# Jeremy-Cleland/hmer-img2latex

Measured on AMD Instinct MI355X. Metric: decoded LaTeX tokens/sec at batch 256, 320x64 imgs, seq 150, higher is better.
Workload: dtype f32

## Files before the change

### hmer-img2latex_amd/csrc/conv_bf16x3.hip

```cpp
#include <stdlib.h>

#include "common.h"

namespace {

#include "bf16_split.inc.h"

typedef float f32x16 __attribute__((ext_vector_type(16)));

constexpr int CH = 16;
constexpr int CO_BLK = 64;
constexpr int W_SLAB_U4 = 9 * 3 * 2 * CO_BLK;
constexpr int W_PHASE_U4 = W_SLAB_U4 / 3;

template <int WX> struct Tile3 {
    static constexpr int TR = (4 / WX) * 4, TC = WX * 16;
    static constexpr int IR = TR + 2, IC = TC + 2;
    static constexpr int ICP = WX == 2 ? 36 : (WX == 1 ? 20 : 68);
    static constexpr int ROW16 = 2 * ICP;
    static constexpr int IN_U4 = 3 * IR * ROW16;
};

constexpr unsigned FIX_HDR = 64;
constexpr unsigned FIX_CAP = 1u << 20;
constexpr float FIX_TOL = 0x1p-13f;

__device__ __forceinline__ void pool_window(float a0, float a1, float a2, float a3, float bv, float& outv, int& bi, bool& near) {
    float best = a0;
    bi = 0;
    if (a1 > best) { best = a1; bi = 1; }
    if (a2 > best) { best = a2; bi = 2; }
    if (a3 > best) { best = a3; bi = 3; }
    const float pre = best + bv;
    outv = fmaxf(pre, 0.f);
    const float scale = fmaxf(fmaxf(fabsf(best), fabsf(bv)), 1e-30f);
    const float thr = FIX_TOL * scale;
    const float d0 = best - a0, d1 = best - a1, d2 = best - a2, d3 = best - a3;
    const bool tie = (d0 > 0.f && d0 <= thr) || (d1 > 0.f && d1 <= thr) || (d2 > 0.f && d2 <= thr) || (d3 > 0.f && d3 <= thr);
    near = fabsf(pre) <= thr || (tie && pre > 0.f);
}
__device__ __forceinline__ void fix_append(unsigned* fix, size_t o) {
    const unsigned at = atomicAdd(fix, 1u);
    if (at < FIX_CAP) fix[FIX_HDR + at] = (unsigned)o;
}

__global__ void conv_pack3_kernel(const float* __restrict__ w, bf16_t* __restrict__ wp, int Cin, int Cout, int n_chunks,
                                  size_t total, int flip, unsigned* __restrict__ fix) {
    const size_t idx = (size_t)blockIdx.x * blockDim.x + threadIdx.x;
    if (idx == 0 && fix) fix[0] = 0;
    if (idx >= total) return;
    size_t r = idx;
    const int j = (int)(r % 8); r /= 8;
    const int co_l = (int)(r % CO_BLK); r /= CO_BLK;
    const int lh = (int)(r % 2); r /= 2;
    const int tap = (int)(r % 9); r /= 9;
    const int chunk = (int)(r % n_chunks);
    const int cb = (int)(r / n_chunks);
    const int co = cb * CO_BLK + co_l, ci = chunk * CH + 8 * lh + j;
    const float v = (co < Cout && ci < Cin) ? (flip ? w[((size_t)ci * Cout + co) * 9 + (8 - tap)] : w[((size_t)co * Cin + ci) * 9 + tap]) : 0.f;
    bf16_t s[3];
    split3(v, s[0], s[1], s[2]);
    const size_t slab = ((size_t)cb * n_chunks + chunk) * (size_t)W_SLAB_U4 * 8;
#pragma unroll
    for (int sp = 0; sp < 3; ++sp)
        wp[slab + ((((size_t)tap * 3 + sp) * 2 + lh) * CO_BLK + co_l) * 8 + j] = s[sp];
}

template <int WX, bool FULL = false, bool AM = false, int NT = 2>
__global__ __launch_bounds__(256, 2) void conv3x3_bf16x3_kernel(
    const float* __restrict__ x, const bf16_t* __restrict__ wpack, const float* __restrict__ bias,
    float* __restrict__ y, unsigned char* __restrict__ amax, int Cin, int H, int W, int Cout, int Hp, int Wp,
    int tiles_x, int n_chunks, int tiles_per_img, int n_items, int items_per_wg, unsigned* __restrict__ fix) {
    typedef Tile3<WX> TL;
    constexpr int PR = TL::TR / 2, PC = TL::TC / 2;
    constexpr bool LO = FULL && NT == 1;
    __shared__ __attribute__((aligned(16))) uint4 in_s[TL::IN_U4];
    __shared__ __attribute__((aligned(16))) uint4 w_s[W_PHASE_U4];
    __shared__ float out_s[CO_BLK * 65];
    __shared__ unsigned char am_s[AM ? CO_BLK * 68 : 4];

    const int tid = threadIdx.x, lane = tid & 63, wave = tid >> 6;
    const int wy = wave / WX, wx = wave % WX;
    constexpr int CO_W = 32 * NT;
    const int co_blocks_g = (Cout + CO_W - 1) / CO_W;
    const int lin = blockIdx.x, within = lin % (8 * co_blocks_g);
    const int cb = within >> 3;
    const int walk = (lin / (8 * co_blocks_g)) * 8 + (within & 7);
    const int i = lane & 31, h = lane >> 5;
    const int dx = i & 1, dy = (i >> 1) & 1, pp = i >> 2;
    const int a_base = ((wy * 4 + dy) * 2 + h) * TL::ICP + wx * 16 + 2 * pp + dx;
    const int b_base = h * CO_BLK + i + (NT == 1 ? (cb & 1) * 32 : 0);
    const uint4* wp_cb = reinterpret_cast<const uint4*>(wpack) + (size_t)(NT == 1 ? cb >> 1 : cb) * n_chunks * W_SLAB_U4;
    const int HW = H * W;

    constexpr int NP = TL::IR * 2 * TL::IC;
    constexpr int NE = (NP + 255) / 256;
    constexpr int NWV = (W_PHASE_U4 + 255) / 256;
    constexpr int SPLIT_U4 = TL::IR * TL::ROW16;
    int loff[NE], p_r[NE], p_col[NE], p_lh[NE];
#pragma unroll
    for (int e = 0; e < NE; ++e) {
        const int idx = tid + e * 256;
        p_col[e] = idx % TL::IC;
        p_lh[e] = (idx / TL::IC) & 1;
        p_r[e] = idx / (2 * TL::IC);
        loff[e] = idx < NP ? (p_r[e] * 2 + p_lh[e]) * TL::ICP + p_col[e] : -1;
    }
    const float* f_xb = x;
    int goff[NE];
    unsigned okmask = 0;
    auto setup_fetch = [&](int item) {
        const int fb = item / tiles_per_img, ft = item - fb * tiles_per_img;
        const int fty = ft / tiles_x, ftx = ft - fty * tiles_x;
        const int fy0 = fty * TL::TR, fx0 = ftx * TL::TC;
        f_xb = x + (size_t)fb * Cin * HW;
        okmask = 0;
#pragma unroll
        for (int e = 0; e < NE; ++e) {
            const int iy = fy0 - 1 + p_r[e], ix = fx0 - 1 + p_col[e];
            goff[e] = (8 * p_lh[e] * H + iy) * W + ix;
            if (loff[e] >= 0 && iy >= 0 && iy < H && ix >= 0 && ix < W) okmask |= 1u << e;
        }
    };
    float xin[NE][8];
    uint4 win[NWV];
    auto fetch_x = [&](int chunk) {
        const float* xc = f_xb + (size_t)chunk * CH * HW;
#pragma unroll
        for (int e = 0; e < NE; ++e) {
            const bool ok = (okmask >> e) & 1u;
#pragma unroll
            for (int j = 0; j < 8; ++j) xin[e][j] = ok ? xc[goff[e] + j * HW] : 0.f;
        }
    };
    auto fetch_w = [&](int phase) {
        const uint4* wsrc = wp_cb + (size_t)phase * W_PHASE_U4;
#pragma unroll
        for (int e = 0; e < NWV; ++e) {
            const int idx = tid + e * 256;
            win[e] = idx < W_PHASE_U4 ? wsrc[idx] : make_uint4(0, 0, 0, 0);
        }
    };
    auto commit_x = [&]() {
#pragma unroll
        for (int e = 0; e < NE; ++e) {
            if (loff[e] >= 0) {
                unsigned s[3][4];
#pragma unroll
                for (int j = 0; j < 4; ++j) split3_pair(xin[e][2 * j], xin[e][2 * j + 1], s[0][j], s[1][j], s[2][j]);
#pragma unroll
                for (int sp = 0; sp < 3; ++sp)
                    in_s[loff[e] + sp * SPLIT_U4] = make_uint4(s[sp][0], s[sp][1], s[sp][2], s[sp][3]);
            }
        }
    };
    auto commit_w = [&]() {
#pragma unroll
        for (int e = 0; e < NWV; ++e) {
            const int idx = tid + e * 256;
            if (idx < W_PHASE_U4) w_s[idx] = win[e];
        }
    };

    const int n_phases = 3 * n_chunks;
    const int it0 = walk * items_per_wg, it_end = min(it0 + items_per_wg, n_items);
    if (it0 >= n_items) return;
    setup_fetch(it0);
    fetch_x(0);
    fetch_w(0);
    for (int it = it0; it < it_end; ++it) {
        const int b = it / tiles_per_img, tl = it - b * tiles_per_img;
        const int ty = tl / tiles_x, tx = tl - ty * tiles_x;
        const int y0 = ty * TL::TR, x0 = tx * TL::TC;
        f32x16 acc[2][NT];
        f32x16 acc_lo[LO ? 2 : 1];
#pragma unroll
        for (int m = 0; m < 2; ++m)
#pragma unroll
            for (int n = 0; n < NT; ++n)
#pragma unroll
                for (int r = 0; r < 16; ++r) acc[m][n][r] = 0.f;
        if constexpr (LO) {
#pragma unroll
            for (int m = 0; m < 2; ++m)
#pragma unroll
                for (int r = 0; r < 16; ++r) acc_lo[m][r] = 0.f;
        }

        for (int chunk = 0; chunk < n_chunks; ++chunk) {
#pragma unroll
            for (int ky = 0; ky < 3; ++ky) {
                __syncthreads();
                if (ky == 0) commit_x();
                commit_w();
                __syncthreads();
                if (chunk * 3 + ky + 1 < n_phases) fetch_w(chunk * 3 + ky + 1);
                else if (it + 1 < it_end) fetch_w(0);
                if (ky == 0) {
                    if (chunk + 1 < n_chunks) fetch_x(chunk + 1);
                    else if (it + 1 < it_end) { setup_fetch(it + 1); fetch_x(0); }
                }
#pragma unroll
                for (int kx = 0; kx < 3; ++kx) {
                    i16x8_t a[2][3], bw[NT][3];
#pragma unroll
                    for (int m = 0; m < 2; ++m)
#pragma unroll
                        for (int sp = 0; sp < 3; ++sp) {
                            const uint4 t = in_s[a_base + (sp * TL::IR + m * 2 + ky) * TL::ROW16 + kx];
                            a[m][sp] = *reinterpret_cast<const i16x8_t*>(&t);
                        }
#pragma unroll
                    for (int n = 0; n < NT; ++n)
#pragma unroll
                        for (int sp = 0; sp < 3; ++sp) {
                            const uint4 t = w_s[b_base + ((kx * 3 + sp) * 2) * CO_BLK + n * 32];
                            bw[n][sp] = *reinterpret_cast<const i16x8_t*>(&t);
                        }
                    constexpr int TI[6] = {0, 1, 2, 0, 1, 0}, TJ[6] = {2, 1, 0, 1, 0, 0};
#pragma unroll
                    for (int t = 0; t < 6; ++t)
#pragma unroll
                        for (int m = 0; m < 2; ++m)
#pragma unroll
                            for (int n = 0; n < NT; ++n) {
                                if constexpr (LO) {
                                    f32x16& dst = t < 5 ? acc_lo[m] : acc[m][n];
                                    dst = __builtin_amdgcn_mfma_f32_32x32x16_bf16(a[m][TI[t]], bw[n][TJ[t]], dst, 0, 0, 0);
                                } else {
                                    acc[m][n] = __builtin_amdgcn_mfma_f32_32x32x16_bf16(a[m][TI[t]], bw[n][TJ[t]], acc[m][n], 0, 0, 0);
                                }
                            }
                }
            }
        }

        const int py0 = y0 >> 1, px0 = x0 >> 1;
        if constexpr (LO) {
#pragma unroll
            for (int m = 0; m < 2; ++m) acc[m][0] += acc_lo[m];
        }
        if constexpr (FULL) {
#pragma unroll
            for (int n = 0; n < NT; ++n) {
                const int co = cb * CO_W + n * 32 + i;
                if (co >= Cout) continue;
#pragma unroll
                for (int m = 0; m < 2; ++m) {
                    const int py = py0 + wy * 2 + m;
#pragma unroll
                    for (int q = 0; q < 4; ++q) {
                        const int px = px0 + wx * 8 + 2 * q + h;
#pragma unroll
                        for (int ry = 0; ry < 2; ++ry) {
                            const int Y = 2 * py + ry, X = 2 * px;
                            if (Y < H && X + 1 < W)
                                *reinterpret_cast<float2*>(y + (((size_t)b * Cout + co) * H + Y) * W + X) =
                                    make_float2(acc[m][n][4 * q + 2 * ry], acc[m][n][4 * q + 2 * ry + 1]);
                        }
                    }
                }
            }
            continue;
        }
        if ((Wp & 3) == 0 && py0 + PR <= Hp && px0 + PC <= Wp && (cb + 1) * CO_BLK <= Cout) {
#pragma unroll
            for (int n = 0; n < NT; ++n) {
                const float bv = bias[cb * CO_BLK + n * 32 + i];
#pragma unroll
                for (int m = 0; m < 2; ++m)
#pragma unroll
                    for (int q = 0; q < 4; ++q) {
                        const int pos = (wy * 2 + m) * PC + wx * 8 + 2 * q + h;
                        if constexpr (AM) {
                            float ov;
                            int bi;
                            bool near;
                            pool_window(acc[m][n][4 * q], acc[m][n][4 * q + 1], acc[m][n][4 * q + 2], acc[m][n][4 * q + 3], bv, ov, bi, near);
                            out_s[(n * 32 + i) * 65 + pos] = ov;
                            am_s[(n * 32 + i) * 68 + pos] = (unsigned char)bi;
                            if (near && fix)
                                fix_append(fix, (((size_t)b * Cout + cb * CO_BLK + n * 32 + i) * Hp + py0 + wy * 2 + m) * Wp + px0 + wx * 8 + 2 * q + h);
                        } else {
                            const float v = fmaxf(fmaxf(acc[m][n][4 * q], acc[m][n][4 * q + 1]),
                                                  fmaxf(acc[m][n][4 * q + 2], acc[m][n][4 * q + 3])) + bv;
                            out_s[(n * 32 + i) * 65 + pos] = fmaxf(v, 0.f);
                        }
                    }
            }
            __syncthreads();
            for (int idx = tid; idx < CO_BLK * 16; idx += 256) {
                constexpr int XG = PC / 4;
                const int x4 = idx % XG, py = (idx / XG) % PR, co_l = idx >> 4;
                const float* sp = &out_s[co_l * 65 + py * PC + 4 * x4];
                const size_t o = (((size_t)b * Cout + cb * CO_BLK + co_l) * Hp + py0 + py) * Wp + px0 + 4 * x4;
                *reinterpret_cast<float4*>(y + o) = make_float4(sp[0], sp[1], sp[2], sp[3]);
                if constexpr (AM) *reinterpret_cast<uchar4*>(amax + o) = *reinterpret_cast<const uchar4*>(&am_s[co_l * 68 + py * PC + 4 * x4]);
            }
            continue;
        }
#pragma unroll
        for (int n = 0; n < NT; ++n) {
            const int co = cb * CO_BLK + n * 32 + i;
            if (co >= Cout) continue;
            const float bv = bias[co];
#pragma unroll
            for (int m = 0; m < 2; ++m) {
                const int py = py0 + wy * 2 + m;
                if (py >= Hp) continue;
                const size_t rowoff = (((size_t)b * Cout + co) * Hp + py) * Wp;
#pragma unroll
                for (int q = 0; q < 4; ++q) {
                    const int px = px0 + wx * 8 + 2 * q + h;
                    float ov;
                    int bi;
                    bool near;
                    pool_window(acc[m][n][4 * q], acc[m][n][4 * q + 1], acc[m][n][4 * q + 2], acc[m][n][4 * q + 3], bv, ov, bi, near);
                    if (px < Wp) {
                        y[rowoff + px] = ov;
                        if (amax) amax[rowoff + px] = (unsigned char)bi;
                        if (AM && near && fix) fix_append(fix, rowoff + px);
                    }
                }
            }
        }
    }
}


template <int CIN, bool AM = false>
__global__ __launch_bounds__(256, 4) void conv3x3_smallk_bf16x3_kernel(
    const float* __restrict__ x, const float* __restrict__ w, const float* __restrict__ bias, float* __restrict__ y,
    unsigned char* __restrict__ amax, int H, int W, int Cout, int Hp, int Wp, int tiles_x, int tiles_per_part,
    unsigned* __restrict__ fix) {
    constexpr int RS = 48;
    constexpr int PLANE = 10 * RS;
    __shared__ __attribute__((aligned(16))) uint2 img[3 * PLANE];
    __shared__ float out_s[32 * 65];
    __shared__ unsigned char am_s[AM ? 32 * 68 : 4];

    const int tid = threadIdx.x, lane = tid & 63, wave = tid >> 6;
    const int wy = wave >> 1, wx = wave & 1;
    const int i = lane & 31, h = lane >> 5;
    const int cbs = (Cout + 31) / 32;
    const int cb = blockIdx.x % cbs, b = blockIdx.z;
    const int tx_begin = (blockIdx.x / cbs) * tiles_per_part, tx_end = min(tiles_x, tx_begin + tiles_per_part);
    const int y0 = blockIdx.y * 8;

    i16x8_t bw[3][3];
    {
        const int co = cb * 32 + i;
#pragma unroll
        for (int s = 0; s < 3; ++s) {
            unsigned pk[3][4];
#pragma unroll
            for (int j = 0; j < 4; ++j) {
                const int tap = 4 * s + 2 * h + (j >> 1), c0 = 2 * (j & 1);
                const bool okt = tap < 9 && co < Cout;
                const float v0 = (okt && c0 < CIN) ? w[((size_t)co * CIN + c0) * 9 + tap] : 0.f;
                const float v1 = (okt && c0 + 1 < CIN) ? w[((size_t)co * CIN + c0 + 1) * 9 + tap] : 0.f;
                split3_pair(v0, v1, pk[0][j], pk[1][j], pk[2][j]);
            }
#pragma unroll
            for (int sp = 0; sp < 3; ++sp) {
                const uint4 t = make_uint4(pk[sp][0], pk[sp][1], pk[sp][2], pk[sp][3]);
                bw[s][sp] = *reinterpret_cast<const i16x8_t*>(&t);
            }
        }
    }
    const float bv = (cb * 32 + i < Cout) ? bias[cb * 32 + i] : 0.f;

    const int pbase = (wy * 4 + ((i >> 1) & 1)) * RS + wx * 16 + 2 * (i >> 2) + (i & 1);
    int aoff[3][2];
#pragma unroll
    for (int s = 0; s < 3; ++s)
#pragma unroll
        for (int e = 0; e < 2; ++e) {
            const int tap = min(4 * s + 2 * h + e, 8);
            aoff[s][e] = pbase + (tap / 3) * RS + (tap % 3);
        }

    const float* xb = x + (size_t)b * CIN * H * W;
    const size_t HW = (size_t)H * W;
    int q_lds[2], q_col[2];
    long q_goff[2];
    bool q_rowok[2];
#pragma unroll
    for (int e = 0; e < 2; ++e) {
        const int q = tid + e * 256;
        const int r = q / 34, col = q - r * 34;
        const int iy = y0 - 1 + r;
        q_lds[e] = q < 340 ? r * RS + col : -1;
        q_col[e] = col - 1;
        q_rowok[e] = q < 340 && iy >= 0 && iy < H;
        q_goff[e] = (long)iy * W + col - 1;
    }
    float pin[2][CIN];
    auto fetch = [&](int tx) {
        const int x0 = tx * 32;
#pragma unroll
        for (int e = 0; e < 2; ++e) {
            const int ix = x0 + q_col[e];
            const bool ok = q_rowok[e] && ix >= 0 && ix < W;
#pragma unroll
            for (int c = 0; c < CIN; ++c) pin[e][c] = ok ? xb[c * HW + q_goff[e] + x0] : 0.f;
        }
    };
    fetch(tx_begin);
    for (int tx = tx_begin; tx < tx_end; ++tx) {
#pragma unroll
        for (int e = 0; e < 2; ++e) {
            if (q_lds[e] >= 0) {
                unsigned p0[3], p1[3];
                split3_pair(pin[e][0], CIN > 1 ? pin[e][CIN > 1 ? 1 : 0] : 0.f, p0[0], p0[1], p0[2]);
                split3_pair(CIN > 2 ? pin[e][CIN > 2 ? 2 : 0] : 0.f, 0.f, p1[0], p1[1], p1[2]);
#pragma unroll
                for (int sp = 0; sp < 3; ++sp) img[sp * PLANE + q_lds[e]] = make_uint2(p0[sp], p1[sp]);
            }
        }
        __syncthreads();
        if (tx + 1 < tx_end) fetch(tx + 1);
#pragma unroll 1
        for (int m = 0; m < 2; ++m) {
            f32x16 acc;
#pragma unroll
            for (int r = 0; r < 16; ++r) acc[r] = 0.f;
            constexpr int TI[5] = {0, 1, 2, 0, 1}, TJ[5] = {2, 1, 0, 1, 0};
            i16x8_t a0[3];
#pragma unroll
            for (int s = 0; s < 3; ++s) {
                i16x8_t a[3];
#pragma unroll
                for (int sp = 0; sp < 3; ++sp) {
                    const uint2 t0 = img[sp * PLANE + m * 2 * RS + aoff[s][0]];
                    const uint2 t1 = img[sp * PLANE + m * 2 * RS + aoff[s][1]];
                    const uint4 t = make_uint4(t0.x, t0.y, t1.x, t1.y);
                    a[sp] = *reinterpret_cast<const i16x8_t*>(&t);
                }
                a0[s] = a[0];
#pragma unroll
                for (int t = 0; t < 5; ++t)
                    acc = __builtin_amdgcn_mfma_f32_32x32x16_bf16(a[TI[t]], bw[s][TJ[t]], acc, 0, 0, 0);
            }
#pragma unroll
            for (int s = 0; s < 3; ++s) acc = __builtin_amdgcn_mfma_f32_32x32x16_bf16(a0[s], bw[s][0], acc, 0, 0, 0);
#pragma unroll
            for (int q = 0; q < 4; ++q) {
                const int pos = (wy * 2 + m) * 16 + wx * 8 + 2 * q + h;
                if constexpr (AM) {
                    float ov;
                    int bi;
                    bool near;
                    pool_window(acc[4 * q], acc[4 * q + 1], acc[4 * q + 2], acc[4 * q + 3], bv, ov, bi, near);
                    out_s[i * 65 + pos] = ov;
                    am_s[i * 68 + pos] = (unsigned char)bi;
                    const int fpy = (y0 >> 1) + wy * 2 + m, fpx = tx * 16 + wx * 8 + 2 * q + h;
                    if (near && fix && cb * 32 + i < Cout && fpy < Hp && fpx < Wp)
                        fix_append(fix, (((size_t)b * Cout + cb * 32 + i) * Hp + fpy) * Wp + fpx);
                } else {
                    const float v = fmaxf(fmaxf(acc[4 * q], acc[4 * q + 1]), fmaxf(acc[4 * q + 2], acc[4 * q + 3])) + bv;
                    out_s[i * 65 + pos] = fmaxf(v, 0.f);
                }
            }
        }
        __syncthreads();
        const int py0 = y0 >> 1, px0 = tx * 16;
        if ((Wp & 3) == 0 && py0 + 4 <= Hp && px0 + 16 <= Wp && (cb + 1) * 32 <= Cout) {
            for (int idx = tid; idx < 32 * 16; idx += 256) {
                const int x4 = idx & 3, py = (idx >> 2) & 3, c = idx >> 4;
                const float* sp = &out_s[c * 65 + py * 16 + 4 * x4];
                const size_t o = (((size_t)b * Cout + cb * 32 + c) * Hp + py0 + py) * Wp + px0 + 4 * x4;
                *reinterpret_cast<float4*>(y + o) = make_float4(sp[0], sp[1], sp[2], sp[3]);
                if constexpr (AM) *reinterpret_cast<uchar4*>(amax + o) = *reinterpret_cast<const uchar4*>(&am_s[c * 68 + py * 16 + 4 * x4]);
            }
        } else {
            for (int idx = tid; idx < 32 * 64; idx += 256) {
                const int px = idx & 15, py = (idx >> 4) & 3, c = idx >> 6;
                if (cb * 32 + c < Cout && py0 + py < Hp && px0 + px < Wp) {
                    const size_t o = (((size_t)b * Cout + cb * 32 + c) * Hp + py0 + py) * Wp + px0 + px;
                    y[o] = out_s[c * 65 + py * 16 + px];
                    if constexpr (AM) amax[o] = am_s[c * 68 + py * 16 + px];
                }
            }
        }
    }
}

__global__ __launch_bounds__(256) void conv_pool_fixup_kernel(const float* __restrict__ x, const float* __restrict__ w,
                                                              const float* __restrict__ bias, float* __restrict__ y,
                                                              unsigned char* __restrict__ amax, const unsigned* __restrict__ fix,
                                                              int Cin, int H, int W, int Cout, int Hp, int Wp) {
    const unsigned n = min(fix[0], FIX_CAP);
    const int lane = threadIdx.x & 63;
    for (unsigned e = blockIdx.x * 4 + (threadIdx.x >> 6); e < n; e += gridDim.x * 4) {
        const unsigned o = fix[FIX_HDR + e];
        const int px = (int)(o % Wp), py = (int)((o / Wp) % Hp);
        const int co = (int)((o / ((unsigned)Wp * Hp)) % Cout), b = (int)(o / ((unsigned)Wp * Hp * Cout));
        float s[4] = {0.f, 0.f, 0.f, 0.f};
        for (int ci = lane; ci < Cin; ci += 64) {
            const float* xp = x + ((size_t)b * Cin + ci) * H * W;
            const float* wp = w + ((size_t)co * Cin + ci) * 9;
            float win[4][4];
#pragma unroll
            for (int r = 0; r < 4; ++r)
#pragma unroll
                for (int c = 0; c < 4; ++c) {
                    const int iy = 2 * py - 1 + r, ix = 2 * px - 1 + c;
                    win[r][c] = (iy >= 0 && iy < H && ix >= 0 && ix < W) ? xp[(size_t)iy * W + ix] : 0.f;
                }
#pragma unroll
            for (int ky = 0; ky < 3; ++ky)
#pragma unroll
                for (int kx = 0; kx < 3; ++kx) {
                    const float wv = wp[ky * 3 + kx];
#pragma unroll
                    for (int q = 0; q < 4; ++q) s[q] = fmaf(win[(q >> 1) + ky][(q & 1) + kx], wv, s[q]);
                }
        }
#pragma unroll
        for (int q = 0; q < 4; ++q)
#pragma unroll
            for (int off = 32; off >= 1; off >>= 1) s[q] += __shfl_xor(s[q], off);
        if (lane == 0) {
            float best = s[0];
            int bi = 0;
#pragma unroll
            for (int q = 1; q < 4; ++q)
                if (s[q] > best) { best = s[q]; bi = q; }
            y[o] = fmaxf(best + bias[co], 0.f);
            amax[o] = (unsigned char)bi;
        }
    }
}

}

bool i2l_conv_bf16x3_applicable(int Cin, int Cout) {
    return Cin % CH == 0 && Cout % CO_BLK == 0;
}
bool i2l_conv_bf16x3_full_applicable(int Cin, int Cout) {
    return Cin % CH == 0 && (Cout % CO_BLK == 0 || Cout == 32);
}

size_t i2l_conv_bf16x3_workspace_bytes(int Cin, int Cout) {
    return i2l_align((size_t)((Cout + CO_BLK - 1) / CO_BLK) * (Cin / CH) * W_SLAB_U4 * 16);
}
size_t i2l_conv_fixlist_bytes(void) { return i2l_align((size_t)(FIX_HDR + FIX_CAP) * sizeof(unsigned)); }

namespace {
int launch_fixup(const float* x, const float* w, const float* bias, float* y, unsigned char* amax, const unsigned* fix,
                 int B, int Cin, int H, int W, int Cout, hipStream_t s) {
    if ((size_t)B * Cout * (H / 2) * (W / 2) > 0xffffffffull) return I2L_ERR_UNSUPPORTED;
    hipLaunchKernelGGL(conv_pool_fixup_kernel, dim3(512), dim3(256), 0, s, x, w, bias, y, amax, fix, Cin, H, W, Cout, H / 2, W / 2);
    I2L_CHECK_LAUNCH();
    return I2L_OK;
}
}

int i2l_conv_bf16x3_run(const float* x, const float* w, const float* bias, float* y, unsigned char* amax, int B, int Cin,
                        int H, int W, int Cout, void* workspace, size_t workspace_bytes, hipStream_t s, int full,
                        int weights_packed) {
    if (full && ((H | W) & 1)) return I2L_ERR_UNSUPPORTED;
    const size_t pack_bytes = i2l_conv_bf16x3_workspace_bytes(Cin, Cout);
    if (workspace_bytes < pack_bytes + (amax ? i2l_conv_fixlist_bytes() : 0) || !workspace) return I2L_ERR_WORKSPACE;
    unsigned* fix = amax ? reinterpret_cast<unsigned*>(static_cast<char*>(workspace) + pack_bytes) : nullptr;
    if (amax && (size_t)B * Cout * (H / 2) * (W / 2) > 0xffffffffull) return I2L_ERR_UNSUPPORTED;
    const int Hp = H / 2, Wp = W / 2;
    const int n_chunks = Cin / CH, co_blocks = (Cout + CO_BLK - 1) / CO_BLK;
    if (Cout % CO_BLK != 0 && !(full && Cout == 32)) return I2L_ERR_UNSUPPORTED;
    bf16_t* wp = static_cast<bf16_t*>(workspace);
    const size_t total = (size_t)co_blocks * n_chunks * 9 * 2 * CO_BLK * 8;
    if (!(weights_packed && !amax && !full))
    hipLaunchKernelGGL(conv_pack3_kernel, dim3((unsigned)((total + 255) / 256)), dim3(256), 0, s, w, wp, Cin, Cout,
                       n_chunks, total, full ? 1 : 0, fix);
    I2L_CHECK_LAUNCH();
    const int rows = 2 * Hp, cols = 2 * Wp;
    int wx = 2;
    long bestw = -1;
    const int cand[3] = {2, 1, 4};
    for (int c = 0; c < 3; ++c) {
        const int tr = (4 / cand[c]) * 4, tc = cand[c] * 16;
        const long cover = (long)i2l_cdiv(rows, tr) * tr * i2l_cdiv(cols, tc) * tc;
        if (bestw < 0 || cover < bestw) { bestw = cover; wx = cand[c]; }
    }
    const int tr = (4 / wx) * 4, tc = wx * 16;
    const int tiles_x = i2l_cdiv(cols, tc), tiles_y = i2l_cdiv(rows, tr);
    const int tiles_per_img = tiles_x * tiles_y;
    const long long n_items_ll = (long long)tiles_per_img * B;
    if (n_items_ll > 0x7fffffffll) return I2L_ERR_UNSUPPORTED;
    const int n_items = (int)n_items_ll;
    const int wg_blocks = full ? (Cout + 31) / 32 : co_blocks;
    int items_per_wg = (int)((n_items_ll * wg_blocks + 511) / 512);
    if (n_items_ll * wg_blocks <= 768) items_per_wg = 1;
    if (items_per_wg < 1) items_per_wg = 1;
    const int walks = i2l_cdiv(n_items, items_per_wg);
    dim3 grid((unsigned)(i2l_cdiv(walks, 8) * 8 * wg_blocks));
#define I2L_LAUNCH3(WXV)                                                                                              \
    do {                                                                                                              \
        if (full)                                                                                                     \
            hipLaunchKernelGGL((conv3x3_bf16x3_kernel<WXV, true, false, 1>), grid, dim3(256), 0, s, x, (const bf16_t*)wp, bias, y, \
                               amax, Cin, H, W, Cout, Hp, Wp, tiles_x, n_chunks, tiles_per_img, n_items, items_per_wg, fix); \
        else if (amax)                                                                                                \
            hipLaunchKernelGGL((conv3x3_bf16x3_kernel<WXV, false, true>), grid, dim3(256), 0, s, x, (const bf16_t*)wp, bias, y, \
                               amax, Cin, H, W, Cout, Hp, Wp, tiles_x, n_chunks, tiles_per_img, n_items, items_per_wg, fix); \
        else                                                                                                          \
            hipLaunchKernelGGL((conv3x3_bf16x3_kernel<WXV, false>), grid, dim3(256), 0, s, x, (const bf16_t*)wp, bias, y, \
                               amax, Cin, H, W, Cout, Hp, Wp, tiles_x, n_chunks, tiles_per_img, n_items, items_per_wg, fix); \
    } while (0)
    if (wx == 2) I2L_LAUNCH3(2);
    else if (wx == 1) I2L_LAUNCH3(1);
    else I2L_LAUNCH3(4);
#undef I2L_LAUNCH3
    I2L_CHECK_LAUNCH();
    if (amax) return launch_fixup(x, w, bias, y, amax, fix, B, Cin, H, W, Cout, s);
    return I2L_OK;
}

bool i2l_conv_smallk_applicable(int Cin, int Cout) {
    return Cin >= 1 && Cin <= 3 && Cout % 32 == 0;
}

int i2l_conv_smallk_run(const float* x, const float* w, const float* bias, float* y, unsigned char* amax, int B, int Cin,
                        int H, int W, int Cout, void* workspace, size_t workspace_bytes, hipStream_t s) {
    const int Hp = H / 2, Wp = W / 2;
    unsigned* fix = nullptr;
    if (amax) {
        if (!workspace || workspace_bytes < i2l_conv_fixlist_bytes()) return I2L_ERR_WORKSPACE;
        if ((size_t)B * Cout * Hp * Wp > 0xffffffffull) return I2L_ERR_UNSUPPORTED;
        fix = static_cast<unsigned*>(workspace);
        if (hipMemsetAsync(fix, 0, sizeof(unsigned), s) != hipSuccess) return I2L_ERR_LAUNCH;
    }
    const int tiles_x = i2l_cdiv(2 * Wp, 32), bands = i2l_cdiv(2 * Hp, 8);
    if (bands > 65535 || B > 65535) return I2L_ERR_UNSUPPORTED;
    int parts = 1;
    while (parts < tiles_x && (long)(Cout / 32) * bands * B * parts < 1536) ++parts;
    const int tiles_per_part = i2l_cdiv(tiles_x, parts);
    parts = i2l_cdiv(tiles_x, tiles_per_part);
    dim3 grid((Cout / 32) * parts, bands, B);
#define I2L_LAUNCH_SK(C, A) hipLaunchKernelGGL((conv3x3_smallk_bf16x3_kernel<C, A>), grid, dim3(256), 0, s, x, w, bias, y, amax, H, W, Cout, Hp, Wp, tiles_x, tiles_per_part, fix)
    if (amax) {
        if (Cin == 1) I2L_LAUNCH_SK(1, true);
        else if (Cin == 2) I2L_LAUNCH_SK(2, true);
        else I2L_LAUNCH_SK(3, true);
    } else {
        if (Cin == 1) I2L_LAUNCH_SK(1, false);
        else if (Cin == 2) I2L_LAUNCH_SK(2, false);
        else I2L_LAUNCH_SK(3, false);
    }
#undef I2L_LAUNCH_SK
    I2L_CHECK_LAUNCH();
    if (amax) return launch_fixup(x, w, bias, y, amax, fix, B, Cin, H, W, Cout, s);
    return I2L_OK;
}
```

Before: 40.57 million.

## Double-buffer conv output tile and defer global store to overlap with MFMA

The output staging buffers (out_s, am_s) are double-buffered so each tile's global store runs during the next tile's MFMA compute rather than serially after it. The last tile is flushed after the loop, and the fast-path store loop is unrolled into two fixed iterations per thread. This adds about 8KB of LDS per block, which may lower occupancy at the requested 4 blocks per CU. Only the small-K first conv layer is affected, which is a small part of the full decode pipeline.

```diff
diff --git a/hmer-img2latex_amd/csrc/conv_bf16x3.hip b/hmer-img2latex_amd/csrc/conv_bf16x3.hip
--- a/hmer-img2latex_amd/csrc/conv_bf16x3.hip
+++ b/hmer-img2latex_amd/csrc/conv_bf16x3.hip
@@ -336,8 +336,8 @@
     constexpr int RS = 48;
     constexpr int PLANE = 10 * RS;
     __shared__ __attribute__((aligned(16))) uint2 img[3 * PLANE];
-    __shared__ float out_s[32 * 65];
-    __shared__ unsigned char am_s[AM ? 32 * 68 : 4];
+    __shared__ float out_s[2][32 * 65];
+    __shared__ unsigned char am_s[2][AM ? 32 * 68 : 4];
 
     const int tid = threadIdx.x, lane = tid & 63, wave = tid >> 6;
     const int wy = wave >> 1, wx = wave & 1;
@@ -406,8 +406,38 @@
             for (int c = 0; c < CIN; ++c) pin[e][c] = ok ? xb[c * HW + q_goff[e] + x0] : 0.f;
         }
     };
+    auto store_tile = [&](int txs, int par) {
+        const int py0 = y0 >> 1, px0 = txs * 16;
+        const float* os = out_s[par];
+        const unsigned char* as = am_s[par];
+        int ts = tid;
+        asm volatile("" : "+v"(ts));
+        if ((Wp & 3) == 0 && py0 + 4 <= Hp && px0 + 16 <= Wp && (cb + 1) * 32 <= Cout) {
+            const int x4 = ts & 3, py = (ts >> 2) & 3;
+            const size_t t = ((size_t)(ts >> 4) * Hp + py) * Wp + 4 * x4;
+#pragma unroll
+            for (int k = 0; k < 2; ++k) {
+                const int c = (ts >> 4) + 16 * k;
+                const float* sp = &os[c * 65 + py * 16 + 4 * x4];
+                const size_t o = (((size_t)b * Cout + cb * 32 + 16 * k) * Hp + py0) * Wp + px0 + t;
+                *reinterpret_cast<float4*>(y + o) = make_float4(sp[0], sp[1], sp[2], sp[3]);
+                if constexpr (AM) *reinterpret_cast<uchar4*>(amax + o) = *reinterpret_cast<const uchar4*>(&as[c * 68 + py * 16 + 4 * x4]);
+            }
+        } else {
+            for (int idx = ts; idx < 32 * 64; idx += 256) {
+                const int px = idx & 15, py = (idx >> 4) & 3, c = idx >> 6;
+                if (cb * 32 + c < Cout && py0 + py < Hp && px0 + px < Wp) {
+                    const size_t o = (((size_t)b * Cout + cb * 32 + c) * Hp + py0 + py) * Wp + px0 + px;
+                    y[o] = os[c * 65 + py * 16 + px];
+                    if constexpr (AM) amax[o] = as[c * 68 + py * 16 + px];
+                }
+            }
+        }
+    };
+    if (tx_begin >= tx_end) return;
     fetch(tx_begin);
     for (int tx = tx_begin; tx < tx_end; ++tx) {
+        const int par = (tx - tx_begin) & 1;
 #pragma unroll
         for (int e = 0; e < 2; ++e) {
             if (q_lds[e] >= 0) {
@@ -420,6 +450,7 @@
         }
         __syncthreads();
         if (tx + 1 < tx_end) fetch(tx + 1);
+        if (tx > tx_begin) store_tile(tx - 1, par ^ 1);
 #pragma unroll 1
         for (int m = 0; m < 2; ++m) {
             f32x16 acc;
@@ -452,38 +483,20 @@
                     int bi;
                     bool near;
                     pool_window(acc[4 * q], acc[4 * q + 1], acc[4 * q + 2], acc[4 * q + 3], bv, ov, bi, near);
-                    out_s[i * 65 + pos] = ov;
-                    am_s[i * 68 + pos] = (unsigned char)bi;
+                    out_s[par][i * 65 + pos] = ov;
+                    am_s[par][i * 68 + pos] = (unsigned char)bi;
                     const int fpy = (y0 >> 1) + wy * 2 + m, fpx = tx * 16 + wx * 8 + 2 * q + h;
                     if (near && fix && cb * 32 + i < Cout && fpy < Hp && fpx < Wp)
                         fix_append(fix, (((size_t)b * Cout + cb * 32 + i) * Hp + fpy) * Wp + fpx);
                 } else {
                     const float v = fmaxf(fmaxf(acc[4 * q], acc[4 * q + 1]), fmaxf(acc[4 * q + 2], acc[4 * q + 3])) + bv;
-                    out_s[i * 65 + pos] = fmaxf(v, 0.f);
+                    out_s[par][i * 65 + pos] = fmaxf(v, 0.f);
                 }
             }
         }
         __syncthreads();
-        const int py0 = y0 >> 1, px0 = tx * 16;
-        if ((Wp & 3) == 0 && py0 + 4 <= Hp && px0 + 16 <= Wp && (cb + 1) * 32 <= Cout) {
-            for (int idx = tid; idx < 32 * 16; idx += 256) {
-                const int x4 = idx & 3, py = (idx >> 2) & 3, c = idx >> 4;
-                const float* sp = &out_s[c * 65 + py * 16 + 4 * x4];
-                const size_t o = (((size_t)b * Cout + cb * 32 + c) * Hp + py0 + py) * Wp + px0 + 4 * x4;
-                *reinterpret_cast<float4*>(y + o) = make_float4(sp[0], sp[1], sp[2], sp[3]);
-                if constexpr (AM) *reinterpret_cast<uchar4*>(amax + o) = *reinterpret_cast<const uchar4*>(&am_s[c * 68 + py * 16 + 4 * x4]);
-            }
-        } else {
-            for (int idx = tid; idx < 32 * 64; idx += 256) {
-                const int px = idx & 15, py = (idx >> 4) & 3, c = idx >> 6;
-                if (cb * 32 + c < Cout && py0 + py < Hp && px0 + px < Wp) {
-                    const size_t o = (((size_t)b * Cout + cb * 32 + c) * Hp + py0 + py) * Wp + px0 + px;
-                    y[o] = out_s[c * 65 + py * 16 + px];
-                    if constexpr (AM) amax[o] = am_s[c * 68 + py * 16 + px];
-                }
-            }
-        }
-    }
+    }
+    store_tile(tx_end - 1, (tx_end - 1 - tx_begin) & 1);
 }
 
 __global__ __launch_bounds__(256) void conv_pool_fixup_kernel(const float* __restrict__ x, const float* __restrict__ w,
```

Result: no change. 40.77 million (median of 2 runs) (+0.5%).
